# zorino/kaamer

Hardware: AMD Instinct MI355X
Metric: k-mer lookups/sec (higher is better)
Workload: dtype u32

## Files before the change

kaamer_amd/csrc/search.hip:

```cpp
#include <hip/hip_runtime.h>

#include <dlfcn.h>

#include <algorithm>
#include <cstdarg>
#include <cstdio>
#include <cstdlib>
#include <cstring>
#include <condition_variable>
#include <memory>
#include <mutex>
#include <new>
#include <vector>

#include "kaamer_internal.h"

static thread_local char g_err[512] = "";

int kaamer_fail(int code, const char *fmt, ...)
{
    va_list ap;
    va_start(ap, fmt);
    vsnprintf(g_err, sizeof g_err, fmt, ap);
    va_end(ap);
// ... 5 lines not shown
        hipError_t e_ = (expr);                                                               \
        if (e_ != hipSuccess)                                                                 \
            return kaamer_fail(KAAMER_E_HIP, "%s failed: %s", #expr, hipGetErrorString(e_)); \
    } while (0)

struct kaamer_workspace;
struct HostSlot {
    kaamer_workspace *ws = nullptr;
    kaamer_workspace_opts opts{};
    uint8_t *d_seqs = nullptr;
    uint64_t *d_off = nullptr;
    size_t seq_cap = 0, off_cap = 0;
    hipStream_t stream = nullptr;
    bool busy = false;
};

static inline bool is_nucl(int32_t seq_type) { return seq_type == KAAMER_NUCLEOTIDE || seq_type == KAAMER_READS; }

struct BatchBounds { uint64_t max_hits, g_slots; uint32_t max_queries; uint32_t pos_scale;  };
static const int MAX_BOUND_RETRIES = 6;

static uint64_t full_start_hits(uint64_t seq_bytes) { return seq_bytes * 8 + 65536; }

static void bounds_grow_positions(BatchBounds &b)
{
    b.pos_scale = b.pos_scale ? (b.pos_scale < (1u << 24) ? b.pos_scale * 4 : b.pos_scale) : 4;
}

static void bounds_grow(BatchBounds &b, uint64_t seq_bytes, uint32_t n_seqs, bool nucl)
{
    b.max_hits = b.max_hits ? b.max_hits * 4 : full_start_hits(seq_bytes);
    b.g_slots = b.g_slots ? b.g_slots * 4 : (128ull << 20);
    if (nucl) {
        const uint64_t hard = seq_bytes / 10 + (uint64_t)n_seqs * 6 + 64;
        b.max_queries = (uint32_t)(hard > 0xFFFFFFF0ull ? 0xFFFFFFF0ull : hard);
    }
    bounds_grow_positions(b);
}

struct TopSlot {
    kaamer_workspace *ws = nullptr;
    kaamer_workspace_opts opts{};
    hipStream_t stream = nullptr;
    uint8_t *d_seqs = nullptr;
    uint64_t *d_off = nullptr;
    size_t seq_cap = 0, off_cap = 0;
    uint8_t *h_in = nullptr;
    size_t h_in_cap = 0;
    uint8_t *d_block = nullptr;
    size_t d_block_cap = 0;
    size_t block_use = 0;
    uint64_t pos_words = 0;
    size_t guess = 1u << 16;
    uint64_t aln_guess = 0;
    bool busy = false;
};
#define KAAMER_MAX_HOST_SLOTS 8
static void top_slot_free(TopSlot &h);

struct kaamer_index {
    int device;
    kh_image_header hdr;
    kh_bucket *d_buckets;
    uint32_t *d_arena;
    HostSlot host[4];
    std::mutex pool_mu;
    std::condition_variable pool_cv;
    TopSlot top[KAAMER_MAX_HOST_SLOTS];
    int n_top;
    uint64_t top_pos_words = 0;
    const kaamer_proteins *aln_host = nullptr;
    uint8_t *d_aln_raw = nullptr, *d_aln_codes = nullptr, *d_aln_bad = nullptr;
    uint64_t *d_aln_off = nullptr;
    uint32_t *d_aln_idmap = nullptr;
    int *d_aln_matrix = nullptr;
    int aln_matrix[26 * 26];
    uint32_t aln_idmap_n = 0, aln_entries = 0, aln_max_ns = 0;
    uint64_t aln_bytes = 0, aln_number_of_aa = 0;
    uint64_t aln_budget = 0;
    uint64_t aln_last[3] = {0, 0, 0};
};

enum { ST_POOL_FULL = 1u, ST_LIST_FULL = 2u, ST_QUERY_CAP = 4u, ST_AA_CAP = 8u, ST_G_ARENA_FULL = 16u, ST_G_TABLE_FULL = 32u,
       ST_POS_UNSUPPORTED = 64u, ST_POS_CAP = 128u, ST_CHAIN_TIMEOUT = 256u, ST_EXCHANGE_CAP = 512u, ST_PEER_FAILED = 1024u,
       ST_IDS_CAP = 2048u ,
       ST_ALN_CAP = 4096u ,
       ST_SEG_CAP = 8192u  };
enum { CTR_IN = 0, CTR_QUERIES, CTR_LOOKUP, CTR_PROBE, CTR_FOUND, CTR_POST, CTR_HITS, CTR_OVERFLOW, CTR_LISTS, CTR_LIST_IDS, CTR_N };
static_assert(sizeof(kaamer_counters) == CTR_N * 8, "counter layout");
#define CTR_REPLICAS 64

enum { LIST_S = 0, LIST_L, LIST_SO, LIST_G, N_LISTS };
enum { SLOT_QUEUE_HEAD = N_LISTS, SLOT_STATUS = N_LISTS + 1, SLOT_GROUP_QUEUE = N_LISTS + 2, SLOT_GROUP_QUEUE_POS = N_LISTS + 3,
       SLOT_N_LONG = N_LISTS + 4, SLOT_TILES_DONE = N_LISTS + 5, SLOT_TR_TICKET = N_LISTS + 6,
       SLOT_QUEUE_SUB = N_LISTS + 7 , SLOT_G_TICKET = N_LISTS + 15, SLOT_PACK_TICKETS = N_LISTS + 16 ,
       SLOT_G_HITS16 = N_LISTS + 80 ,
       SLOT_G_MON_HITS16 = N_LISTS + 81 , SLOT_G_MONSTERS = N_LISTS + 82 ,
       N_SMALL_SLOTS = N_LISTS + 16 + 64 + 3 };
#define G_MONSTER_HITS (GRP_MAX_TABLE / 4u * 3u)
static_assert(N_SMALL_SLOTS <= 256, "the finalize step zeroes one slot per thread");
struct alignas(16) WorkItem {
    uint32_t q;
    int32_t size;
    uint64_t aa_off;
};

#define CURSOR_STRIDE 32u
#define MAX_TIMED_CALLS 1024u
#define L_WAVES 8
#define L_LOG2CAP 12
#define G_WAVES 8
#ifndef S_MIN_WAVES
#define S_MIN_WAVES 1
#endif
#ifndef L_MIN_WAVES
#define L_MIN_WAVES 1
#endif
#ifndef S_NWIN
#define S_NWIN 3
#endif

__device__ __forceinline__ uint32_t lane_id() { return threadIdx.x & 63u; }

__device__ __forceinline__ uint32_t wave_sum32(uint32_t v)
{
#pragma unroll
    for (int o = 32; o > 0; o >>= 1) v += __shfl_xor(v, o, 64);
    return v;
}
__device__ __forceinline__ uint32_t wave_total(uint32_t v)
{
    return (uint32_t)__builtin_amdgcn_readfirstlane((int)wave_sum32(v));
}

__device__ __forceinline__ void add_counter(unsigned long long *replicas, uint32_t replica, int which, unsigned long long v)
{
    if (v) atomicAdd(&replicas[(size_t)(replica % CTR_REPLICAS) * CTR_N + which], v);
}

struct ProbeParams {
    const uint4 *table;
    uint64_t n_buckets;
    uint32_t n_shards, shard;
    const uint8_t *residues;
    unsigned long long *invalid;
    const unsigned long long *d_n_pos;
    uint32_t *vals;
    unsigned long long *counters;
    uint32_t nontemporal;
};

#define P_WAVES 4
#define P_RING 128u
#define KH_NO_KEY 0xFFFFFFFDu

template <bool SKIP_IDLE> __global__ __launch_bounds__(64 * P_WAVES) void probe_kernel(ProbeParams p)
{
    __shared__ uint8_t s_lut[256];
    __shared__ uint8_t s_stage[P_WAVES][80];
    __shared__ uint32_t s_ring[P_WAVES][3][P_RING];
    const uint32_t tid = threadIdx.x, lane = tid & 63u;
    const uint32_t wv = (uint32_t)__builtin_amdgcn_readfirstlane((int)(tid >> 6));
    const unsigned long long n_pos = *p.d_n_pos;
    const unsigned long long n_win = (n_pos + 63) >> 6;
    for (uint32_t i = tid; i < 256; i += 64 * P_WAVES) s_lut[i] = (uint8_t)kh_residue_code((uint8_t)i);
    __syncthreads();
    uint32_t c_lookup = 0, c_probe = 0, c_found = 0;
    uint8_t *stage = s_stage[wv];
    uint32_t *const ring_key = s_ring[wv][0], *const ring_pos = s_ring[wv][1], *const ring_step = s_ring[wv][2];
    uint32_t ring_head = 0, ring_n = 0;
    const uint32_t n_buckets = (uint32_t)p.n_buckets;
    const uint32_t mine = 16u * (lane & 3u) + (lane >> 2);

    const unsigned long long stride = (unsigned long long)gridDim.x * P_WAVES;
    unsigned long long w = (unsigned long long)blockIdx.x * P_WAVES + wv;
    unsigned long long mask = 0;
    uint32_t ra = 0, rb = 0;
    auto fetch = [&](unsigned long long win, unsigned long long &m, uint32_t &a, uint32_t &b) {
        const unsigned long long wc = win < n_win ? win : n_win - 1;
        m = p.invalid[wc];
        const unsigned long long i0 = (wc << 6) + lane, last = n_pos - 1;
        a = p.residues[i0 < last ? i0 : last];
        b = p.residues[i0 + 64 < last ? i0 + 64 : last];
    };
    if (n_win) fetch(w, mask, ra, rb);

    while (n_win) {
        const bool ring = ring_n >= 64u || (w >= n_win && ring_n > 0u);
        if (!ring && w >= n_win) break;
        unsigned long long base = 0;
        uint32_t key = KH_NO_KEY, off = lane, step = 0;
        if (ring) {
            const uint32_t n = ring_n < 64u ? ring_n : 64u;
            if (lane < n) {
                const uint32_t slot = (ring_head + lane) & (P_RING - 1u);
                key = ring_key[slot]; off = ring_pos[slot]; step = ring_step[slot];
            }
            ring_head = (ring_head + n) & (P_RING - 1u);
            ring_n -= n;
        } else {
            base = w << 6;
            stage[lane] = s_lut[ra];
            if (lane < 6) stage[64 + lane] = s_lut[rb];
            __builtin_amdgcn_fence(__ATOMIC_ACQ_REL, "wavefront");
            __builtin_amdgcn_wave_barrier();
            const uint8_t *st = stage + lane;
            key = kh_key_from_codes(st[0], st[1], st[2], st[3], st[4], st[5], st[6]);
            const bool own = p.n_shards <= 1 || kh_shard_of(key, p.n_shards) == p.shard;
            key = (((~mask >> lane) & 1ull) && own) ? key : KH_NO_KEY;
            __builtin_amdgcn_fence(__ATOMIC_ACQ_REL, "wavefront");
            __builtin_amdgcn_wave_barrier();
            c_lookup += key != KH_NO_KEY ? 1u : 0u;
        }
        c_probe += key != KH_NO_KEY ? 1u : 0u;
        const unsigned long long w_cur = w;
        if (!ring) w += stride;
        fetch(w, mask, ra, rb);

        uint32_t my_bucket = 0u;
        if (key != KH_NO_KEY) {
            my_bucket = (uint32_t)kh_home_bucket(key, p.n_shards, p.n_buckets) + step;
            my_bucket = my_bucket >= n_buckets ? my_bucket - n_buckets : my_bucket;
        }
        uint4 ld[4];
        uint32_t rk[4];
#pragma unroll
        for (int j = 0; j < 4; j++) {
            const int src = 16 * j + (int)(lane >> 2);
            rk[j] = __shfl(key, src, 64);
            const uint32_t bucket = __shfl(my_bucket, src, 64);
            typedef uint32_t v4u __attribute__((ext_vector_type(4)));
            const v4u *srcp = reinterpret_cast<const v4u *>(p.table) + (uint64_t)bucket * 4 + (lane & 3u);
            if (SKIP_IDLE) {
                ld[j] = make_uint4(KH_EMPTY_KEY, 0u, KH_EMPTY_KEY, 0u);
                if (rk[j] != KH_NO_KEY) {
                    const v4u t = *srcp;
                    ld[j] = make_uint4(t.x, t.y, t.z, t.w);
                }
            } else {
                const v4u t = p.nontemporal ? __builtin_nontemporal_load(srcp) : *srcp;
                ld[j] = make_uint4(t.x, t.y, t.z, t.w);
            }
        }
        uint32_t okey = KH_NO_KEY, oval = 0, oempty = 1u;
#pragma unroll
        for (int j = 0; j < 4; j++) {
            const uint32_t kk = rk[j];
            uint32_t r = (ld[j].x == kk) ? ld[j].y : ((ld[j].z == kk) ? ld[j].w : 0u);
            uint32_t e = (ld[j].x == KH_EMPTY_KEY || ld[j].z == KH_EMPTY_KEY) ? 1u : 0u;
            r |= (uint32_t)__builtin_amdgcn_update_dpp(0, (int)r, 0xB1, 0xf, 0xf, false);
            e |= (uint32_t)__builtin_amdgcn_update_dpp(0, (int)e, 0xB1, 0xf, 0xf, false);
            r |= (uint32_t)__builtin_amdgcn_update_dpp(0, (int)r, 0x4E, 0xf, 0xf, false);
            e |= (uint32_t)__builtin_amdgcn_update_dpp(0, (int)e, 0x4E, 0xf, 0xf, false);
            const bool take = (lane & 3u) == (uint32_t)j;
            okey = take ? kk : okey; oval = take ? r : oval; oempty = take ? e : oempty;
        }
        const uint32_t ooff = __shfl(off, (int)mine, 64);
        const bool valid = okey != KH_NO_KEY;
        c_found += (valid && oval != 0u) ? 1u : 0u;
        const unsigned long long W = __ballot(valid && oval == 0u && oempty == 0u);
        if (W) {
            const uint32_t ostep = __shfl(step, (int)mine, 64);
            const bool wk = valid && oval == 0u && oempty == 0u && ostep + 1u < n_buckets;
            const unsigned long long W2 = __ballot(wk);
            if (wk) {
                const uint32_t slot = (ring_head + ring_n + (uint32_t)__builtin_amdgcn_mbcnt_hi((uint32_t)(W2 >> 32), __builtin_amdgcn_mbcnt_lo((uint32_t)W2, 0u))) & (P_RING - 1u);
                ring_key[slot] = okey;
                ring_pos[slot] = (uint32_t)base + ooff;
                ring_step[slot] = ostep + 1u;
            }
            ring_n += (uint32_t)__popcll(W2);
        }
        __builtin_amdgcn_fence(__ATOMIC_ACQ_REL, "wavefront");
        __builtin_amdgcn_wave_barrier();
        if (!ring || oval != 0u) p.vals[base + ooff] = oval;
        if (lane == 0) p.invalid[ring ? n_win + 1 : w_cur] = 0ull;
    }
    const uint32_t t_lookup = wave_total(c_lookup), t_probe = wave_total(c_probe), t_found = wave_total(c_found);
    if (lane == 0) {
        const uint32_t rep = blockIdx.x * P_WAVES + wv;
        add_counter(p.counters, rep, CTR_LOOKUP, t_lookup);
        add_counter(p.counters, rep, CTR_PROBE, t_probe);
        add_counter(p.counters, rep, CTR_FOUND, t_found);
    }
}

struct QInfo;
struct CountParams {
    const uint32_t *arena;
    const uint32_t *vals;
    const struct QInfo *qinfo;
    const uint64_t *slot_off;
    uint32_t *group_first;
    const uint32_t *d_n_groups;
    const uint32_t *d_nq;
    uint32_t last_group_pass;
    uint32_t pack_shift;
    uint32_t *pack_tickets;
    const uint64_t *pos_base;
    unsigned long long *pos_bits;
    const uint32_t *m_pid, *m_km, *m_fp;
    uint32_t merge_fp;
    const WorkItem *list;
    const uint32_t *list_count;
    WorkItem *ovf_list;
    uint32_t *ovf_count;
    uint32_t list_cap;
    uint32_t *queue_head;
    uint32_t *group_queue;
    const uint2 *sched;
    const uint32_t *d_n_sched;
    uint64_t *hit_off;
    uint32_t *q_cnt;
    uint32_t *hit_pid, *hit_km, *hit_fp;
    uint64_t hit_cap;
    unsigned long long *tail_cursor;
    uint32_t *g_keys;
    uint64_t g_slots;
    unsigned long long *g_cursor;
    uint32_t n_proteins;
    unsigned long long *counters;
    uint32_t *status;
    kaamer_counters *fin_out;
    uint32_t *fin_small, *fin_status_out;
    unsigned long long *fin_cursors;
    uint32_t *fin_slot_scale;
    uint32_t fin_scale_cap, fin_scale_margin;
};

__device__ __forceinline__ unsigned long long tail_alloc(const CountParams &p, uint32_t total)
{
    const unsigned long long b = p.slot_off[*p.d_nq] + atomicAdd(p.tail_cursor, (unsigned long long)total);
    if (b + total > p.hit_cap) { atomicOr(p.status, (uint32_t)ST_POOL_FULL); return ~0ull; }
    return b;
}

template <int LOG2CAP, bool FIRSTPOS = true> struct LdsTable {
    volatile uint32_t *keys;
    uint32_t *cnt, *minpos, *nd;
    static constexpr uint32_t CAP = 1u << LOG2CAP;
    static constexpr uint32_t LIMIT = CAP - CAP / 4;
    __device__ __forceinline__ bool add_n(uint32_t pid, uint32_t pos, uint32_t n, uint32_t &nnew) const
    {
        constexpr uint32_t MASK = CAP - 1u;
        uint32_t h = (pid * 0x9E3779B1u) >> (32 - LOG2CAP);
        for (uint32_t t = 0; t <= MASK; t++) {
            uint32_t k = keys[h];
            if (k == KH_EMPTY_PID) {
                const uint32_t old = atomicCAS((uint32_t *)&keys[h], KH_EMPTY_PID, pid);
                if (old == KH_EMPTY_PID) { nnew++; k = pid; }
                else k = old;
            }
            if (k == pid) {
                atomicAdd(&cnt[h], n);
                if (FIRSTPOS) atomicMin(&minpos[h], pos);
                return true;
            }
            h = (h + 1u) & MASK;
        }
        return false;
    }
    __device__ __forceinline__ bool over_limit() const { return *(volatile uint32_t *)nd > LIMIT; }
};

#define BIG_LOG2CAP 13
struct BigLdsTable {
    uint32_t *keys, *val, *nd;
    static constexpr uint32_t CAP = 1u << BIG_LOG2CAP;
    static constexpr uint32_t LIMIT = CAP - CAP / 4;
    __device__ __forceinline__ bool add_n(uint32_t pid, uint32_t pos, uint32_t n, uint32_t &nnew) const
    {
        uint32_t h = (pid * 0x9E3779B1u) >> (32 - BIG_LOG2CAP);
        for (uint32_t t = 0; t < 128u; t++) {
            uint32_t k = __hip_atomic_load(&keys[h], __ATOMIC_RELAXED, __HIP_MEMORY_SCOPE_WORKGROUP);
            if (k == KH_EMPTY_PID) {
                const uint32_t old = atomicCAS(&keys[h], KH_EMPTY_PID, pid);
                if (old == KH_EMPTY_PID) { k = pid; if (atomicAdd(nd, 1u) >= LIMIT) return false; }
                else k = old;
            }
            if (k == pid) {
                atomicAdd(&val[h], n);
                uint32_t old = __hip_atomic_load(&val[h], __ATOMIC_RELAXED, __HIP_MEMORY_SCOPE_WORKGROUP);
                while (pos < (old >> 16)) {
                    const uint32_t seen = atomicCAS(&val[h], old, (old & 0xFFFFu) | (pos << 16));
                    if (seen == old) break;
                    old = seen;
                }
                return true;
            }
            h = (h + 1u) & (CAP - 1u);
        }
        return false;
    }
    __device__ __forceinline__ bool over_limit() const { return false; }
};

#define G_MAX_RANGES 64u
__device__ __forceinline__ uint32_t g_range_of(uint32_t pid, uint32_t R) { return (uint32_t)(((uint64_t)(pid * 0x85EBCA6Bu) * R) >> 32); }
struct RangeHist {
    uint32_t *cnt, *nd;
    uint32_t R;
    __device__ __forceinline__ bool add_n(uint32_t pid, uint32_t, uint32_t, uint32_t &) const { atomicAdd(&cnt[g_range_of(pid, R)], 1u); return true; }
    __device__ __forceinline__ bool over_limit() const { return false; }
};
struct RangeScatter {
    uint32_t *cur, *nd;
    uint2 *items;
    uint32_t R;
    const uint32_t *first;
    uint32_t cap;
    uint32_t *ovf;
    __device__ __forceinline__ bool add_n(uint32_t pid, uint32_t pos, uint32_t n, uint32_t &) const
    {
        const uint32_t r = g_range_of(pid, R);
        const uint32_t at = atomicAdd(&cur[r], 1u);
        if (at - first[r] < cap) items[at] = make_uint2(pid, pos | (n << 16));
        else *ovf = 1u;
        return true;
    }
    __device__ __forceinline__ bool over_limit() const { return false; }
};

struct GlobalTable {
    uint32_t *slots;
    uint32_t *nd;
    uint32_t log2cap;
    __device__ __forceinline__ bool add_n(uint32_t pid, uint32_t pos, uint32_t n, uint32_t &nnew) const
    {
        const uint32_t mask = (1u << log2cap) - 1u;
// ... 1398 lines not shown
    if (!rc) rc = dev_alloc(&ws->d_counter_replicas, (size_t)CTR_REPLICAS * CTR_N);
    if (!rc) rc = dev_alloc(&ws->d_counters, 1);
    if (!rc) rc = dev_alloc(&ws->d_bsum, ws->n_scan_blocks);
    if (!rc) rc = dev_alloc(&ws->d_chain, (size_t)ws->q_cap / PL_TILE + 2);
    if (!rc && hipMemset(ws->d_chain, 0, ((size_t)ws->q_cap / PL_TILE + 2) * sizeof(unsigned long long)) != hipSuccess) rc = kaamer_fail(KAAMER_E_HIP, "memset");
    if (!rc) rc = dev_alloc(&ws->d_hit_off, (size_t)ws->q_cap + 1);
    ws->compact = opts->compact != 0;
    if (!rc) rc = dev_alloc(&ws->d_hit_pid, ws->sparse_cap);
    if (!rc) rc = dev_alloc(&ws->d_hit_km, ws->sparse_cap);
    if (!rc) rc = dev_alloc(&ws->d_hit_fp, ws->sparse_cap);
    if (!rc && !ws->firstpos && hipMemset(ws->d_hit_fp, 0, ws->sparse_cap * sizeof(uint32_t)) != hipSuccess) rc = kaamer_fail(KAAMER_E_HIP, "memset");
    if (!rc && ws->compact) {
        rc = dev_alloc(&ws->d_csr_off, (size_t)ws->q_cap + 1);
        if (!rc) rc = dev_alloc(&ws->d_c_pid, ws->hit_cap);
        if (!rc) rc = dev_alloc(&ws->d_c_km, ws->hit_cap);
        if (!rc) rc = dev_alloc(&ws->d_c_fp, ws->hit_cap);
        if (!rc && !ws->firstpos && hipMemset(ws->d_c_fp, 0, ws->hit_cap * sizeof(uint32_t)) != hipSuccess) rc = kaamer_fail(KAAMER_E_HIP, "memset");
    }
    if (rc) { kaamer_workspace_free(ws); return rc; }
    ws->ev = new (std::nothrow) std::vector<hipEvent_t>();
    if (!ws->ev) { kaamer_workspace_free(ws); return kaamer_fail(KAAMER_E_NOMEM, "event ring"); }
    *out = ws;
    return KAAMER_OK;
}

static void launch_layout(kaamer_workspace *ws, uint32_t nq_bound, uint32_t *status, hipStream_t s, uint32_t bshift, bool schedule = true)
{
    const uint32_t cshift = bshift > GRP_SHIFT ? 10u : bshift >= GRP_SHIFT ? 9u : 7u;
    const uint32_t tiles = (uint32_t)(((uint64_t)nq_bound + 1 + LAY_TILE - 1) / LAY_TILE);
    hipLaunchKernelGGL(layout_kernel, dim3(tiles), dim3(LAY_THREADS), 0, s, ws->d_slots, ws->d_nq, ws->d_slot_off, ws->d_group_first,
                       ws->d_group_start, ws->d_n_groups, ws->groups_cap, ws->d_chain, next_epoch(ws->lay_epoch), status, bshift);
    if (schedule)
        hipLaunchKernelGGL(schedule_kernel, dim3(1), dim3(1024), 0, s, ws->d_group_first, ws->d_group_start, ws->d_slot_off, ws->d_n_groups,
                           ws->d_nq, ws->d_sched, ws->d_n_sched, cshift);
}

static void launch_pos_layout(kaamer_workspace *ws, uint32_t nq_bound, const int32_t *sizes, uint32_t *status, hipStream_t s)
{
    uint32_t gb = (nq_bound + 255) / 256;
    if (gb < 1) gb = 1;
    if (gb > (uint32_t)ws->n_cu * 8) gb = (uint32_t)ws->n_cu * 8;
    hipLaunchKernelGGL(pos_words_kernel, dim3(gb), dim3(256), 0, s, ws->d_qinfo, sizes, ws->d_q_cnt, ws->d_nq, ws->d_pos_words);
    scan_u32_on(ws, ws->d_pos_words, ws->d_nq, nq_bound, ws->d_pos_base, s);
    hipLaunchKernelGGL(pos_layout_kernel, dim3(ws->n_cu * 8), dim3(256), 0, s, ws->d_qinfo, sizes, ws->d_q_cnt,
                       ws->compact ? ws->d_csr_off : ws->d_hit_off,
                       ws->d_pos_base, ws->d_nq, ws->d_pos_off, ws->d_pos_bits, ws->bits_cap, status);
}

static void launch_compaction(kaamer_workspace *ws, uint32_t nq_bound, uint32_t *status, hipStream_t s)
{
    scan_u32_on(ws, ws->d_q_cnt, ws->d_nq, nq_bound, ws->d_csr_off, s);
    uint32_t gb = (nq_bound + 3) / 4;
    if (gb < 1) gb = 1;
    if (gb > (uint32_t)ws->n_cu * 8) gb = (uint32_t)ws->n_cu * 8;
    hipLaunchKernelGGL(gather_hits_kernel, dim3(gb), dim3(256), 0, s, ws->d_nq, ws->d_csr_off, ws->d_hit_off, ws->d_q_cnt, ws->d_hit_pid,
                       ws->d_hit_km, ws->d_hit_fp, ws->d_c_pid, ws->d_c_km, ws->d_c_fp, ws->hit_cap, status, 1);
}

static void fill_result_hits(const kaamer_workspace *ws, kaamer_device_result *out)
{
    out->d_hit_cnt = ws->d_q_cnt;
    out->hit_capacity = ws->compact ? ws->hit_cap : ws->sparse_cap;
    out->d_hit_off = ws->compact ? ws->d_csr_off : ws->d_hit_off;
    out->d_hit_pid = ws->compact ? ws->d_c_pid : ws->d_hit_pid;
    out->d_hit_kmatch = ws->compact ? ws->d_c_km : ws->d_hit_km;
    out->d_hit_first_pos = ws->compact ? ws->d_c_fp : ws->d_hit_fp;
}

static int ws_join(kaamer_workspace *ws, hipStream_t stream)
{
    if (ws->split_pending && ws->count_stream && ws->count_stream != stream) HIPCHK(hipStreamWaitEvent(stream, ws->ev_count, 0));
    return KAAMER_OK;
}

int kaamer_workspace_set_count_stream(kaamer_workspace *ws, void *stream)
{
    if (!ws) return kaamer_fail(KAAMER_E_ARG, "workspace_set_count_stream: bad argument");
    HIPCHK(hipSetDevice(ws->device));
    if (ws->split_pending) HIPCHK(hipEventSynchronize(ws->ev_count));
    ws->split_pending = false;
    ws->count_stream = (hipStream_t)stream;
    if (stream && !ws->ev_probe) {
        HIPCHK(hipEventCreateWithFlags(&ws->ev_probe, hipEventDisableTiming));
        HIPCHK(hipEventCreateWithFlags(&ws->ev_count, hipEventDisableTiming));
    }
    return KAAMER_OK;
}


static void enqueue_protein_prep(kaamer_workspace *ws, const uint8_t *d_seqs, const uint64_t *d_offsets, uint32_t n_seqs, uint64_t seq_bytes,
                                 uint32_t *status, hipStream_t s)
{
    PrepLayoutParams pl;
    memset(&pl, 0, sizeof pl);
    pl.seqs = d_seqs; pl.pos_bound = seq_bytes; pl.offsets = d_offsets; pl.n_seqs = n_seqs;
    pl.q = ws->d_q; pl.d_nq = ws->d_nq; pl.d_n_pos = ws->d_n_pos; pl.invalid = ws->d_valid; pl.qinfo = ws->d_qinfo;
    pl.hit_off = ws->d_hit_off; pl.q_cnt = ws->d_q_cnt;
    pl.E = ws->d_slot_off; pl.group_first = ws->d_group_first; pl.group_start = ws->d_group_start;
    pl.d_n_groups = ws->d_n_groups; pl.groups_cap = ws->groups_cap; pl.chain = ws->d_chain;
    pl.epoch = next_epoch(ws->lay_epoch);
    pl.status = status; pl.sched = ws->d_sched; pl.d_n_sched = ws->d_n_sched;
    pl.tiles_done = ws->d_list_counts + SLOT_TILES_DONE;
    pl.slots = ws->d_slots; pl.bshift = ws->pack_shift; pl.cshift = ws->pack_shift > GRP_SHIFT ? 10u : ws->pack_shift >= GRP_SHIFT ? 9u : 7u;
    pl.no_sched = 0u;
    pl.d_total = ws->d_lay_total;
    pl.slot_scale = ws->d_slot_scale;
    pl.room_slots = ws->table_room;
    const uint32_t tiles = (uint32_t)(((uint64_t)n_seqs + 1 + PL_TILE - 1) / PL_TILE);
    hipLaunchKernelGGL(prep_layout_schedule_kernel, dim3(tiles), dim3(LAY_THREADS), 0, s, pl);
}

struct QueryInput {
    const uint8_t *residues;
    uint64_t pos_bound;
    uint32_t nq_bound;
};

static QueryInput enqueue_translate(kaamer_workspace *ws, const uint8_t *d_seqs, const uint64_t *d_offsets, uint32_t n_seqs, uint64_t seq_bytes,
                                    uint32_t *status, hipStream_t s)
{
    const size_t cap6 = (size_t)ws->max_seqs * 6;
    TranslateParams tp;
    memset(&tp, 0, sizeof tp);
    tp.seqs = d_seqs; tp.offsets = d_offsets; tp.n_seqs = n_seqs; tp.seq_bound = seq_bytes; tp.max_long = ws->max_long; tp.max_piece_items = ws->max_piece_items;
    tp.cnt_orf = ws->d_cnt3; tp.cnt_aa = ws->d_cnt3 + cap6; tp.cnt_sa = ws->d_cnt3 + 2 * cap6;
    tp.off_orf = ws->d_off3; tp.off_aa = ws->d_off3 + (cap6 + 1); tp.off_sa = ws->d_off3 + 2 * (cap6 + 1);
    tp.tmp_meta = ws->d_tmp_meta; tp.orf_aa = ws->d_orf_aa; tp.starts_alt = ws->d_starts_alt;
    tp.q_cap = ws->q_cap; tp.aa_cap = ws->aa_cap; tp.sa_cap = ws->sa_cap; tp.status = status;
    const bool wide_reads = ws->wide_reads >= 0 ? ws->wide_reads != 0 : seq_bytes > 160ull * (n_seqs ? n_seqs : 1u);
    tp.ts_max = wide_reads ? TS_MAX_WIDE : TS_MAX;
    int tgrid = ws->n_cu * 8;
    tp.d_n6 = ws->d_n6;
    int sgrid = ws->n_cu * 8;
    if ((uint64_t)sgrid * TS_WAVES * 64 > (uint64_t)n_seqs) sgrid = n_seqs > 0 ? (int)(((uint64_t)n_seqs + TS_WAVES * 64 - 1) / (TS_WAVES * 64)) : 1;
    tp.n_long = ws->d_list_counts + SLOT_N_LONG;
    const size_t mpi = (size_t)ws->max_piece_items;
    tp.long_seq = ws->d_long_seq; tp.long_np = ws->d_long_np; tp.piece_base = ws->d_piece_base; tp.piece_li = ws->d_piece_li;
    tp.pcnt_orf = ws->d_pcnt3; tp.pcnt_aa = ws->d_pcnt3 + mpi; tp.pcnt_sa = ws->d_pcnt3 + 2 * mpi;
    tp.poff_orf = ws->d_poff3; tp.poff_aa = ws->d_poff3 + (mpi + 1); tp.poff_sa = ws->d_poff3 + 2 * (mpi + 1);
    tp.d_n_piece_items = ws->d_n_piece_items;
    const uint64_t long_bound = (uint64_t)ws->max_long < n_seqs ? ws->max_long : n_seqs;
    const uint64_t seq_long_max = seq_bytes / (TS_MAX + 1) + 1;
    const uint64_t n_long_bound = long_bound < seq_long_max ? long_bound : seq_long_max;
    const uint64_t piece_bound = 6ull * (seq_bytes / 3 / TP_PIECE + n_long_bound + 1);
    if ((uint64_t)tgrid * 4 > piece_bound) tgrid = (int)((piece_bound + 3) / 4);
    if (tgrid < 1) tgrid = 1;
    tp.ticket = ws->d_list_counts + SLOT_TR_TICKET;
    tp.chain = ws->d_tr_chain;
    tp.epoch = next_epoch(ws->tr_epoch);
    tp.out_meta = ws->d_q; tp.d_nq = ws->d_nq; tp.d_n_pos = ws->d_n_pos;
    tp.w_off_orf = ws->d_off3; tp.w_off_aa = ws->d_off3 + (cap6 + 1); tp.w_off_sa = ws->d_off3 + 2 * (cap6 + 1);
    hipLaunchKernelGGL(list_long_kernel, dim3((unsigned)(((uint64_t)n_seqs + LL_BLOCK - 1) / LL_BLOCK + (n_seqs ? 0 : 1))), dim3(LL_BLOCK), 0, s, tp);
    scan_u32_on(ws, ws->d_long_np, tp.n_long, n_long_bound, ws->d_piece_base, s);
    hipLaunchKernelGGL(piece_li_kernel, dim3((unsigned)((n_long_bound + 255) / 256)), dim3(256), 0, s, tp);
    hipLaunchKernelGGL(translate_kernel<false>, dim3(tgrid), dim3(256), 0, s, tp);
    for (int a = 0; a < 3; a++) scan_u32_on(ws, ws->d_pcnt3 + a * mpi, ws->d_n_piece_items, piece_bound, ws->d_poff3 + a * (mpi + 1), s);
    hipLaunchKernelGGL(long_totals_kernel, dim3((unsigned)((n_long_bound * 6 + 255) / 256)), dim3(256), 0, s, tp);
    if (wide_reads) hipLaunchKernelGGL(translate_reads_kernel<TS_MAX_WIDE>, dim3(sgrid), dim3(64 * TS_WAVES), 0, s, tp);
    else hipLaunchKernelGGL(translate_reads_kernel<TS_MAX>, dim3(sgrid), dim3(64 * TS_WAVES), 0, s, tp);
    hipLaunchKernelGGL(translate_kernel<true>, dim3(tgrid), dim3(256), 0, s, tp);
    hipLaunchKernelGGL(orf_order_long_kernel, dim3((unsigned)(n_long_bound < (uint64_t)ws->n_cu * 32 ? (n_long_bound + 3) / 4 + 1 : (uint64_t)ws->n_cu * 8)), dim3(256), 0, s,
                       ws->d_tmp_meta, tp.off_orf, ws->d_long_seq, tp.n_long, ws->d_q, ws->d_nq);
    hipLaunchKernelGGL(prep_orf_kernel, dim3(ws->n_cu * 4), dim3(256), 0, s, ws->d_q, ws->d_nq, ws->d_valid, ws->d_n_pos,
                       ws->d_qinfo, ws->d_slots, ws->d_hit_off, ws->d_q_cnt, ws->d_slot_scale, ws->table_room);
    return QueryInput{ ws->d_orf_aa, ws->aa_cap, ws->q_cap };
}

static void enqueue_probe(const kaamer_index *ix, kaamer_workspace *ws, const uint8_t *residues, uint64_t pos_bound, hipStream_t s)
{
    ProbeParams pp;
    pp.table = reinterpret_cast<const uint4 *>(ix->d_buckets);
    pp.n_buckets = ix->hdr.n_buckets;
    pp.n_shards = ix->hdr.n_shards;
    pp.shard = ix->hdr.shard;
    pp.residues = residues;
    pp.invalid = ws->d_valid;
    pp.d_n_pos = ws->d_n_pos;
    pp.vals = ws->d_vals;
    pp.counters = ws->d_counter_replicas;
    pp.nontemporal = pos_bound < ix->hdr.n_buckets ? 1u : 0u;
    uint64_t p_blocks = (pos_bound / 64 + 1 + P_WAVES - 1) / P_WAVES;
    if (p_blocks > (uint64_t)ws->p_grid) p_blocks = ws->p_grid;
    if (p_blocks < 1) p_blocks = 1;
    if (ws->nucleotide) hipLaunchKernelGGL(probe_kernel<true>, dim3((unsigned)p_blocks), dim3(64 * P_WAVES), 0, s, pp);
    else hipLaunchKernelGGL(probe_kernel<false>, dim3((unsigned)p_blocks), dim3(64 * P_WAVES), 0, s, pp);
}

static CountParams search_count_params(const kaamer_index *ix, const kaamer_workspace *ws)
{
    CountParams p = count_params_base(ws);
    p.arena = ix->d_arena;
    p.vals = ws->d_vals;
    p.queue_head = ws->d_list_counts + SLOT_QUEUE_HEAD;
    p.n_proteins = ix->hdr.max_protein_id + 1u ? ix->hdr.max_protein_id + 1u : 0xFFFFFFFFu;
    return p;
}

static bool fused_finalize(const kaamer_workspace *ws) { return !ws->compact && !ws->want_positions; }

static void enqueue_count(const kaamer_index *ix, kaamer_workspace *ws, bool nucl, uint64_t seq_bytes, uint32_t n_seqs, uint32_t nq_bound,
                          uint64_t pos_bound, hipStream_t s)
{
    const CountParams p = search_count_params(ix, ws);
    CountParams pc = p;
    pc.ovf_list = ws_list(ws, LIST_G); pc.ovf_count = ws->d_list_counts + LIST_G;
    pc.last_group_pass = ws->want_positions ? 0u : 1u;
    pc.pack_shift = ws->pack_shift;
    pc.pack_tickets = ws->d_list_counts + SLOT_PACK_TICKETS;
    if (!nucl) {
        launch_group(pc, group_grid(ws, nq_bound, pos_bound), ws->firstpos, s);
    } else {
        uint64_t gb = (((uint64_t)GRP_MIN_TABLE * nq_bound + 3 * pos_bound) >> ws->pack_shift) + 1;
        if (gb > (uint64_t)ws->pack_grid) gb = ws->pack_grid;
        const bool long_orfs = seq_bytes > 200ull * (n_seqs ? n_seqs : 1u) || ws->dense_tables;
        if (long_orfs) {
            if (gb > (uint64_t)ws->pack_grid_long) gb = ws->pack_grid_long;
            hipLaunchKernelGGL((count_pack_kernel<PK_ARENA_ORF_LONG>), dim3((unsigned)gb), dim3(64), 0, s, pc);
        } else {
            hipLaunchKernelGGL((count_pack_kernel<PK_ARENA_ORF>), dim3((unsigned)gb), dim3(64), 0, s, pc);
        }
    }
    CountParams pg = p;
    pg.list = ws_list(ws, LIST_G); pg.list_count = ws->d_list_counts + LIST_G;
    if (fused_finalize(ws)) {
        pg.fin_out = ws->d_counters; pg.fin_small = ws->d_list_counts; pg.fin_status_out = ws->d_status_out;
        pg.fin_cursors = ws->d_pool_cursor;
        pg.fin_slot_scale = ws->d_slot_scale; pg.fin_scale_cap = ws->slot_scale_cap; pg.fin_scale_margin = ws->slot_scale_margin;
    }
    hipLaunchKernelGGL(count_global_kernel, dim3(g_tier_grid(ws, nq_bound)), dim3(64 * G_WAVES), 0, s, pg);
    if (ws->compact) launch_compaction(ws, nq_bound, p.status, s);
}

static void enqueue_positions(const kaamer_index *ix, kaamer_workspace *ws, uint32_t nq_bound, uint64_t pos_bound, hipStream_t s)
{
    const CountParams p = search_count_params(ix, ws);
    launch_pos_layout(ws, nq_bound, nullptr, p.status, s);
    launch_layout(ws, nq_bound, p.status, s, GRP_SHIFT);
    CountParams pp2 = p;
    pp2.pack_shift = GRP_SHIFT;
    pp2.last_group_pass = 1u;
    pp2.pos_base = ws->d_pos_base;
    pp2.pos_bits = ws->d_pos_bits;
    pp2.group_queue = ws->d_list_counts + SLOT_GROUP_QUEUE_POS;
    pp2.ovf_list = ws_list(ws, LIST_SO); pp2.ovf_count = ws->d_list_counts + LIST_SO;
    launch_group_positions(pp2, group_grid(ws, nq_bound, pos_bound), s);
    CountParams pg2 = p;
    pg2.list = ws_list(ws, LIST_G); pg2.list_count = ws->d_list_counts + LIST_G;
    pg2.pos_base = ws->d_pos_base;
    pg2.pos_bits = ws->d_pos_bits;
    pg2.g_cursor = ws->d_pool_cursor + 2 * CURSOR_STRIDE;
    hipLaunchKernelGGL(positions_global_kernel, dim3(g_tier_grid(ws, nq_bound)), dim3(64 * G_WAVES), 0, s, pg2);
}

int kaamer_search_device(kaamer_index *ix, kaamer_workspace *ws, const uint8_t *d_seqs, const uint64_t *d_offsets,
                         uint32_t n_seqs, uint64_t seq_bytes, int32_t seq_type, void *stream,
                         kaamer_device_result *out)
{
    if (!ix || !ws || !out || (n_seqs && (!d_seqs || !d_offsets))) return kaamer_fail(KAAMER_E_ARG, "search_device: bad argument");
    if (ix->device != ws->device) return kaamer_fail(KAAMER_E_ARG, "workspace belongs to another device");
    const bool nucl = is_nucl(seq_type);
    if (!nucl && seq_type != KAAMER_PROTEIN) return kaamer_fail(KAAMER_E_ARG, "search_device: unknown sequence type %d", seq_type);
    if (nucl != ws->nucleotide) return kaamer_fail(KAAMER_E_ARG, "workspace was created for %s input", ws->nucleotide ? "nucleotide" : "protein");
    if (n_seqs > ws->max_seqs) return kaamer_fail(KAAMER_E_CAPACITY, "batch of %u sequences exceeds workspace max_seqs %u", n_seqs, ws->max_seqs);
    if (ws->pos_cap > 0xFFFFFFF0ull) return kaamer_fail(KAAMER_E_CAPACITY, "a batch holds at most 2^32 residue positions");
    if (seq_bytes > ws->opts.max_seq_bytes) return kaamer_fail(KAAMER_E_CAPACITY, "batch of %llu bytes exceeds workspace max_seq_bytes", (unsigned long long)seq_bytes);
    hipStream_t s = (hipStream_t)stream;
    HIPCHK(hipSetDevice(ix->device));
    {
        const int jrc = ws_join(ws, s);
        if (jrc) return jrc;
        ws->split_pending = false;
    }
    const bool timed = ws->time_every && (ws->call_no++ % ws->time_every) == 0;
    hipEvent_t *ev = nullptr;
    if (timed) {
        if (ws->n_timed >= MAX_TIMED_CALLS) ws->n_timed = 0;
        while (ws->ev->size() < (size_t)(ws->n_timed + 1) * EV_PER_CALL) {
            hipEvent_t e;
            HIPCHK(hipEventCreate(&e));
            ws->ev->push_back(e);
        }
        ev = ws->ev->data() + (size_t)ws->n_timed * EV_PER_CALL;
        HIPCHK(hipEventRecord(ev[0], s));
    }
    {
        const int rrc = ws_reset_if_dirty(ws, s);
        if (rrc) return rrc;
        ws->clean = false;
    }
    uint32_t *status = ws->d_list_counts + SLOT_STATUS;

    QueryInput qin = { d_seqs, seq_bytes, n_seqs };
    if (!nucl) {
        enqueue_protein_prep(ws, d_seqs, d_offsets, n_seqs, seq_bytes, status, s);
    } else {
        qin = enqueue_translate(ws, d_seqs, d_offsets, n_seqs, seq_bytes, status, s);
        launch_layout(ws, qin.nq_bound, status, s, ws->pack_shift, false);
    }
    if (timed) HIPCHK(hipEventRecord(ev[1], s));
    enqueue_probe(ix, ws, qin.residues, qin.pos_bound, s);
    if (timed) HIPCHK(hipEventRecord(ev[2], s));
    const bool split = ws->count_stream && ws->count_stream != s && !timed;
    if (split) {
        HIPCHK(hipEventRecord(ws->ev_probe, s));
        HIPCHK(hipStreamWaitEvent(ws->count_stream, ws->ev_probe, 0));
        s = ws->count_stream;
    }
    enqueue_count(ix, ws, nucl, seq_bytes, n_seqs, qin.nq_bound, qin.pos_bound, s);
    if (timed) HIPCHK(hipEventRecord(ev[3], s));
    if (ws->want_positions) enqueue_positions(ix, ws, qin.nq_bound, qin.pos_bound, s);
// ... 1005 lines not shown
```

Before: 26.95 billion.

## Hand off leftover probe rings to last wave in workgroup

```diff
diff --git a/kaamer_amd/csrc/search.hip b/kaamer_amd/csrc/search.hip
--- a/kaamer_amd/csrc/search.hip
+++ b/kaamer_amd/csrc/search.hip
@@ -181,52 +181,90 @@
 
 #define P_WAVES 4
 #define P_RING 128u
+#define P_HO (P_WAVES * 3u * P_RING)
+#define P_HO_STRIDE (P_WAVES * 64u)
+#define P_Q_WORDS (P_HO + 3u * P_HO_STRIDE)
 #define KH_NO_KEY 0xFFFFFFFDu
 
 template <bool SKIP_IDLE> __global__ __launch_bounds__(64 * P_WAVES) void probe_kernel(ProbeParams p)
 {
     __shared__ uint8_t s_lut[256];
     __shared__ uint8_t s_stage[P_WAVES][80];
-    __shared__ uint32_t s_ring[P_WAVES][3][P_RING];
+    __shared__ uint32_t s_q[P_Q_WORDS];
+    __shared__ uint32_t s_left[P_WAVES], s_arrived;
     const uint32_t tid = threadIdx.x, lane = tid & 63u;
     const uint32_t wv = (uint32_t)__builtin_amdgcn_readfirstlane((int)(tid >> 6));
-    const unsigned long long n_pos = *p.d_n_pos;
-    const unsigned long long n_win = (n_pos + 63) >> 6;
+    const uint32_t n_pos = (uint32_t)*p.d_n_pos;
+    const uint32_t n_win = (n_pos >> 6) + ((n_pos & 63u) ? 1u : 0u);
     for (uint32_t i = tid; i < 256; i += 64 * P_WAVES) s_lut[i] = (uint8_t)kh_residue_code((uint8_t)i);
+    if (tid == 0) s_arrived = 0u;
     __syncthreads();
     uint32_t c_lookup = 0, c_probe = 0, c_found = 0;
     uint8_t *stage = s_stage[wv];
-    uint32_t *const ring_key = s_ring[wv][0], *const ring_pos = s_ring[wv][1], *const ring_step = s_ring[wv][2];
+    const uint32_t ring_at = wv * 3u * P_RING;
+    uint32_t *const ring_key = s_q + ring_at, *const ring_pos = ring_key + P_RING, *const ring_step = ring_pos + P_RING;
     uint32_t ring_head = 0, ring_n = 0;
+    bool is_last = false;
+    uint32_t ho_left = 0, ho_done = 0, ho_1 = 0, ho_2 = 0, ho_3 = 0;
     const uint32_t n_buckets = (uint32_t)p.n_buckets;
     const uint32_t mine = 16u * (lane & 3u) + (lane >> 2);
 
-    const unsigned long long stride = (unsigned long long)gridDim.x * P_WAVES;
-    unsigned long long w = (unsigned long long)blockIdx.x * P_WAVES + wv;
+    const uint32_t stride = gridDim.x * P_WAVES;
+    uint32_t w = blockIdx.x * P_WAVES + wv;
     unsigned long long mask = 0;
     uint32_t ra = 0, rb = 0;
-    auto fetch = [&](unsigned long long win, unsigned long long &m, uint32_t &a, uint32_t &b) {
-        const unsigned long long wc = win < n_win ? win : n_win - 1;
+    auto fetch = [&](uint32_t win, unsigned long long &m, uint32_t &a, uint32_t &b) {
+        const uint32_t wc = win < n_win ? win : n_win - 1u;
         m = p.invalid[wc];
-        const unsigned long long i0 = (wc << 6) + lane, last = n_pos - 1;
-        a = p.residues[i0 < last ? i0 : last];
-        b = p.residues[i0 + 64 < last ? i0 + 64 : last];
+        const uint32_t i0 = (wc << 6) | lane, end = n_pos - 1u;
+        a = p.residues[i0 < end ? i0 : end];
+        b = p.residues[i0 < end && end - i0 > 64u ? i0 + 64u : end];
     };
     if (n_win) fetch(w, mask, ra, rb);
 
-    while (n_win) {
-        const bool ring = ring_n >= 64u || (w >= n_win && ring_n > 0u);
-        if (!ring && w >= n_win) break;
-        unsigned long long base = 0;
+    for (;;) {
+        const bool have = w < n_win;
+        if (!have && ring_n < 64u && !is_last) {
+            if (lane < ring_n) {
+                const uint32_t slot = (ring_head + lane) & (P_RING - 1u), at = P_HO + wv * 64u + lane;
+                s_q[at] = ring_key[slot]; s_q[at + P_HO_STRIDE] = ring_pos[slot]; s_q[at + 2u * P_HO_STRIDE] = ring_step[slot];
+            }
+            if (lane == 0) s_left[wv] = ring_n;
+            __builtin_amdgcn_fence(__ATOMIC_RELEASE, "workgroup", "local");
+            uint32_t before = 0;
+            if (lane == 0) before = __hip_atomic_fetch_add(&s_arrived, 1u, __ATOMIC_RELAXED, __HIP_MEMORY_SCOPE_WORKGROUP);
+            if ((uint32_t)__builtin_amdgcn_readfirstlane((int)before) != P_WAVES - 1u) break;
+            __builtin_amdgcn_fence(__ATOMIC_ACQUIRE, "workgroup", "local");
+            is_last = true;
+            ring_head = ring_n = 0;
+            ho_1 = (uint32_t)__builtin_amdgcn_readfirstlane((int)s_left[0]);
+            ho_2 = ho_1 + (uint32_t)__builtin_amdgcn_readfirstlane((int)s_left[1]);
+            ho_3 = ho_2 + (uint32_t)__builtin_amdgcn_readfirstlane((int)s_left[2]);
+            ho_left = ho_3 + (uint32_t)__builtin_amdgcn_readfirstlane((int)s_left[3]);
+        }
+        const bool from_ho = ring_n < 64u && ho_left > 0u;
+        const bool ring = ring_n >= 64u || from_ho || (is_last && ring_n > 0u);
+        if (!ring && !have) break;
+        uint32_t base = 0;
         uint32_t key = KH_NO_KEY, off = lane, step = 0;
         if (ring) {
-            const uint32_t n = ring_n < 64u ? ring_n : 64u;
-            if (lane < n) {
-                const uint32_t slot = (ring_head + lane) & (P_RING - 1u);
-                key = ring_key[slot]; off = ring_pos[slot]; step = ring_step[slot];
+            uint32_t n, at, fs;
+            if (from_ho) {
+                n = ho_left < 64u ? ho_left : 64u;
+                const uint32_t e = ho_done + lane;
+                const uint32_t seg = (e >= ho_1 ? 1u : 0u) + (e >= ho_2 ? 1u : 0u) + (e >= ho_3 ? 1u : 0u);
+                at = P_HO + seg * 64u + (e - (e >= ho_3 ? ho_3 : e >= ho_2 ? ho_2 : e >= ho_1 ? ho_1 : 0u));
+                fs = P_HO_STRIDE;
+                ho_done += n;
+                ho_left -= n;
+            } else {
+                n = ring_n < 64u ? ring_n : 64u;
+                at = ring_at + ((ring_head + lane) & (P_RING - 1u));
+                fs = P_RING;
+                ring_head = (ring_head + n) & (P_RING - 1u);
+                ring_n -= n;
             }
-            ring_head = (ring_head + n) & (P_RING - 1u);
-            ring_n -= n;
+            if (lane < n) { key = s_q[at]; off = s_q[at + fs]; step = s_q[at + 2u * fs]; }
         } else {
             base = w << 6;
             stage[lane] = s_lut[ra];
@@ -242,7 +280,7 @@
             c_lookup += key != KH_NO_KEY ? 1u : 0u;
         }
         c_probe += key != KH_NO_KEY ? 1u : 0u;
-        const unsigned long long w_cur = w;
+        const uint32_t w_cur = w;
         if (!ring) w += stride;
         fetch(w, mask, ra, rb);
 
@@ -295,7 +333,7 @@
             if (wk) {
                 const uint32_t slot = (ring_head + ring_n + (uint32_t)__builtin_amdgcn_mbcnt_hi((uint32_t)(W2 >> 32), __builtin_amdgcn_mbcnt_lo((uint32_t)W2, 0u))) & (P_RING - 1u);
                 ring_key[slot] = okey;
-                ring_pos[slot] = (uint32_t)base + ooff;
+                ring_pos[slot] = base + ooff;
                 ring_step[slot] = ostep + 1u;
             }
             ring_n += (uint32_t)__popcll(W2);
@@ -303,7 +341,7 @@
         __builtin_amdgcn_fence(__ATOMIC_ACQ_REL, "wavefront");
         __builtin_amdgcn_wave_barrier();
         if (!ring || oval != 0u) p.vals[base + ooff] = oval;
-        if (lane == 0) p.invalid[ring ? n_win + 1 : w_cur] = 0ull;
+        if (lane == 0) p.invalid[ring ? n_win + 1u : w_cur] = 0ull;
     }
     const uint32_t t_lookup = wave_total(c_lookup), t_probe = wave_total(c_probe), t_found = wave_total(c_found);
     if (lane == 0) {
@@ -2008,10 +2046,10 @@
     tp.w_off_orf = ws->d_off3; tp.w_off_aa = ws->d_off3 + (cap6 + 1); tp.w_off_sa = ws->d_off3 + 2 * (cap6 + 1);
     hipLaunchKernelGGL(list_long_kernel, dim3((unsigned)(((uint64_t)n_seqs + LL_BLOCK - 1) / LL_BLOCK + (n_seqs ? 0 : 1))), dim3(LL_BLOCK), 0, s, tp);
     scan_u32_on(ws, ws->d_long_np, tp.n_long, n_long_bound, ws->d_piece_base, s);
-    hipLaunchKernelGGL(piece_li_kernel, dim3((unsigned)((n_long_bound + 255) / 256)), dim3(256), 0, s, tp);
+    hipLaunchKernelGGL(piece_li_kernel, dim3((unsigned)((n_long_bound + 255) / 256 + (n_long_bound ? 0 : 1))), dim3(256), 0, s, tp);
     hipLaunchKernelGGL(translate_kernel<false>, dim3(tgrid), dim3(256), 0, s, tp);
     for (int a = 0; a < 3; a++) scan_u32_on(ws, ws->d_pcnt3 + a * mpi, ws->d_n_piece_items, piece_bound, ws->d_poff3 + a * (mpi + 1), s);
-    hipLaunchKernelGGL(long_totals_kernel, dim3((unsigned)((n_long_bound * 6 + 255) / 256)), dim3(256), 0, s, tp);
+    hipLaunchKernelGGL(long_totals_kernel, dim3((unsigned)((n_long_bound * 6 + 255) / 256 + (n_long_bound ? 0 : 1))), dim3(256), 0, s, tp);
     if (wide_reads) hipLaunchKernelGGL(translate_reads_kernel<TS_MAX_WIDE>, dim3(sgrid), dim3(64 * TS_WAVES), 0, s, tp);
     else hipLaunchKernelGGL(translate_reads_kernel<TS_MAX>, dim3(sgrid), dim3(64 * TS_WAVES), 0, s, tp);
     hipLaunchKernelGGL(translate_kernel<true>, dim3(tgrid), dim3(256), 0, s, tp);
```

Result: no change. 27.00 billion (median of 5 runs) (+0.2%).
